# yoffy/libiqo

Hardware: AMD Instinct MI355X
Metric: Mpix/s Lanczos-3 U8 4K→1080p at 1/2/4/8 GPUs; achieved HBM GB/s %peak (higher is better)
Workload: dtype u8; 1 GPU; C2 Lanczos-3 U8 1ch 3840x2160->1920x1080; frames_per_gpu=1024, global_frames=1024, parallelism=image-sharded x1 (independent shards, no collective), kernel=lanczos_stream, bands_per_frame=auto, step=one libiqo_hip launch over the rank's device-resident batch

## Files before the change

### include/iqo_hip.h

```cpp
#ifndef IQO_HIP_H
#define IQO_HIP_H

#include <stddef.h>
#include <stdint.h>

#ifdef __cplusplus
extern "C" {
#endif

#define IQO_HIP_OK 0
#define IQO_HIP_EINVAL (-1)
#define IQO_HIP_ENODEV (-2)
#define IQO_HIP_ENOMEM (-3)
#define IQO_HIP_EHIP (-4)
#define IQO_HIP_EUNSUP (-5)

enum { IQO_METHOD_LANCZOS = 0, IQO_METHOD_AREA = 1, IQO_METHOD_LINEAR = 2 };

enum {
    IQO_KERNEL_GENERAL = 0,
    IQO_KERNEL_LANCZOS_STREAM = 1,
    IQO_KERNEL_AREA_INT = 2,
    IQO_KERNEL_LINEAR_UP2 = 3,
    IQO_KERNEL_TILE = 4,
// ... 145 lines not shown
int iqo_host_packed_kernel_for(int method, unsigned degree, int channels, size_t srcW, size_t srcH, size_t dstW,
                               size_t dstH, size_t pxScale);

enum {
    IQO_YUV420_NONE = 0,
    IQO_YUV420_LZ_SYMB10 = 1,
    IQO_YUV420_LZ_SYM10 = 2,
    IQO_YUV420_LZ_SYMB8 = 3,
    IQO_YUV420_LZ_SYM8 = 4,
    IQO_YUV420_AREA44 = 5,
    IQO_YUV420_AREA22 = 6,
    IQO_YUV420_AREA2Y = 7,
    IQO_YUV420_AREA4Y = 8,
    IQO_YUV420_AREA8Y = 9,
    IQO_YUV420_AREA33 = 10,
    IQO_YUV420_AREA3Y = 11,
    IQO_YUV420_AREA6Y = 12,
    IQO_YUV420_LIN_D2 = 13,
    IQO_YUV420_LIN_UP2 = 14
};

int iqo_host_yuv420_fused(int method, unsigned degree, size_t srcW, size_t srcH, size_t dstW, size_t dstH);

void iqo_dropin_backend_counts(int *hip, int *cpu);

#ifdef __cplusplus
}
#endif
#endif
```

### libiqo_amd/__init__.py

```python
import ctypes
import os

__all__ = ["IqoError", "LanczosResizer", "AreaResizer", "LinearResizer", "Yuv420Resizer", "Nv12Resizer", "available",
           "lib", "host_tables", "host_kernel_for", "host_packed_kernel_for", "host_yuv420_fused", "host_band_src_rows", "copy_frames", "ipc_export", "ipc_open",
           "ipc_close", "KERNELS", "YUV420_FUSED", "COPY_PATHS", "LIB_PATH", "Norm", "OUT_F32", "OUT_F16", "OUT_BF16",
           "CS_BT601_LIMITED", "CS_BT601_FULL", "CS_BT709_LIMITED", "CS_BT709_FULL", "COLOR_STANDARDS", "RGB_ORDERS",
           "host_yuv_to_rgb", "yuv_rgb_workspace_bytes", "CHROMA_REPLICATE", "CHROMA_FULL", "CHROMA_MODES",
           "host_chroma_full_kernel"]

PKG_DIR = os.path.dirname(os.path.abspath(__file__))
LIB_PATH = os.environ.get("LIBIQO_AMD_LIB") or os.path.join(PKG_DIR, "libiqo_hip.so")

KERNELS = {0: "general", 1: "lanczos_stream", 2: "area_int", 3: "linear_up2", 4: "tile", 5: "walk", 6: "lanczos_up2", 7: "lanczos_d32", 8: "area_d32", 9: "lanczos_u23", 10: "linear_u23", 11: "lanczos_d31", 12: "ryx", 13: "ryg", 14: "packed_tile", 15: "packed_general"}
YUV420_FUSED = {0: "none", 1: "lz_symb10", 2: "lz_sym10", 3: "lz_symb8", 4: "lz_sym8", 5: "area44", 6: "area22",
                7: "area2y", 8: "area4y", 9: "area8y", 10: "area33", 11: "area3y", 12: "area6y", 13: "lin_d2",
                14: "lin_up2"}
_METHODS = {"lanczos": 0, "area": 1, "linear": 2}

_c_sz = ctypes.c_size_t
_vp = ctypes.c_void_p


class IqoError(RuntimeError):
    pass


class PlanDesc(ctypes.Structure):
    _fields_ = [("method", ctypes.c_int), ("device", ctypes.c_int), ("srcW", _c_sz), ("srcH", _c_sz),
                ("dstW", _c_sz), ("dstH", _c_sz), ("tapsX", ctypes.c_int), ("tapsY", ctypes.c_int),
                ("phasesX", ctypes.c_int), ("phasesY", ctypes.c_int), ("kernel", ctypes.c_int),
                ("bandsPerFrame", ctypes.c_int), ("tileRows", ctypes.c_int)]


class Norm(ctypes.Structure):
    _fields_ = [("dtype", ctypes.c_int), ("planes", ctypes.c_int), ("order", ctypes.c_int * 4),
                ("scale", ctypes.c_float * 4), ("bias", ctypes.c_float * 4)]


OUT_F32, OUT_F16, OUT_BF16 = 1, 2, 3
CS_BT601_LIMITED, CS_BT601_FULL, CS_BT709_LIMITED, CS_BT709_FULL = 0, 1, 2, 3
COLOR_STANDARDS = {"bt601": CS_BT601_LIMITED, "bt601-full": CS_BT601_FULL, "bt709": CS_BT709_LIMITED,
                   "bt709-full": CS_BT709_FULL}
RGB_ORDERS = {"rgb": (0, 1, 2), "bgr": (2, 1, 0), "rgba": (0, 1, 2, 3), "bgra": (2, 1, 0, 3)}
CHROMA_REPLICATE, CHROMA_FULL = 0, 1
CHROMA_MODES = {"replicate": CHROMA_REPLICATE, "full": CHROMA_FULL}


class IpcHandle(ctypes.Structure):
    _fields_ = [("bytes", ctypes.c_ubyte * 64), ("offset", ctypes.c_uint64)]


COPY_PATHS = {0: "same device", 1: "peer DMA (xGMI)", 2: "host staging", 3: "host<->device"}

_lib = None
# ... 25 lines not shown
                                             _vp, _vp]
    L.iqo_hip_band_src_rows.argtypes = [_vp, _c_sz, _c_sz, ctypes.POINTER(_c_sz), ctypes.POINTER(_c_sz)]
    L.iqo_hip_resize_band.argtypes = [_vp, _c_sz, _c_sz, _c_sz, _c_sz, _c_sz, _c_sz, _vp, _c_sz, _c_sz, _vp, _vp]
    L.iqo_hip_strerror.restype = ctypes.c_char_p
    L.iqo_hip_strerror.argtypes = [ctypes.c_int]
    L.iqo_hip_version.restype = ctypes.c_char_p
    L.iqo_host_tables.argtypes = [ctypes.c_int, ctypes.c_uint, _c_sz, _c_sz, _c_sz, _c_sz, _c_sz, ctypes.c_int,
                                  ctypes.POINTER(ctypes.c_int), ctypes.POINTER(ctypes.c_int),
                                  ctypes.POINTER(ctypes.c_int32), _c_sz]
    L.iqo_host_kernel_for.argtypes = [ctypes.c_int, ctypes.c_uint, _c_sz, _c_sz, _c_sz, _c_sz, _c_sz]
    L.iqo_host_kernel_for_layout.argtypes = L.iqo_host_kernel_for.argtypes + [_c_sz, _c_sz]
    L.iqo_host_band_src_rows.argtypes = [ctypes.c_int, ctypes.c_uint, _c_sz, _c_sz, _c_sz, _c_sz, _c_sz, _c_sz, _c_sz,
                                         ctypes.POINTER(_c_sz), ctypes.POINTER(_c_sz)]
    L.iqo_hip_plan_yuv420.argtypes = [ctypes.c_int, ctypes.c_uint, _c_sz, _c_sz, _c_sz, _c_sz, ctypes.c_int, pp]
    L.iqo_hip_yuv_plan_destroy.argtypes = [_vp]
    L.iqo_hip_yuv_plan_destroy.restype = None
    L.iqo_hip_yuv_plane.argtypes = [_vp, ctypes.c_int]
    L.iqo_hip_yuv_plane.restype = _vp
    L.iqo_hip_resize_yuv420_device.argtypes = [_vp, _c_sz, _c_sz, _c_sz, _c_sz, _vp, _vp, _vp, _c_sz, _c_sz, _c_sz,
                                               _vp, _vp, _vp, _vp, ctypes.POINTER(ctypes.c_int)]
    L.iqo_hip_resize_yuv420.argtypes = [_vp, _c_sz, _vp, _c_sz, _vp, _vp, _c_sz, _vp, _c_sz, _vp, _vp]
    L.iqo_host_packed_kernel_for.argtypes = [ctypes.c_int, ctypes.c_uint, ctypes.c_int, _c_sz, _c_sz, _c_sz, _c_sz, _c_sz]
    L.iqo_host_yuv420_fused.argtypes = [ctypes.c_int, ctypes.c_uint, _c_sz, _c_sz, _c_sz, _c_sz]
    L.iqo_hip_plan_nv12.argtypes = [ctypes.c_int, ctypes.c_uint, _c_sz, _c_sz, _c_sz, _c_sz, ctypes.c_int, pp]
    L.iqo_hip_nv12_plan_destroy.argtypes = [_vp]
    L.iqo_hip_nv12_plan_destroy.restype = None
    L.iqo_hip_nv12_plane.argtypes = [_vp, ctypes.c_int]
    L.iqo_hip_nv12_plane.restype = _vp
    L.iqo_hip_resize_nv12_device.argtypes = [_vp, _c_sz, _c_sz, _c_sz, _c_sz, _vp, _vp, _c_sz, _c_sz, _c_sz, _vp, _vp,
                                             _vp]
    src_nv12 = [_vp, _c_sz, _c_sz, _c_sz, _c_sz, _vp, _vp]
    src_i420 = src_nv12 + [_vp]
    to_rgb = [ctypes.c_int, ctypes.c_int, ctypes.POINTER(ctypes.c_int), _c_sz, _c_sz, _vp, _vp, _c_sz, _vp]
    to_norm = [ctypes.c_int, ctypes.POINTER(Norm), _c_sz, _c_sz, _c_sz, _vp, _vp, _c_sz, _vp]
    L.iqo_hip_yuv_rgb_workspace_bytes.argtypes = [_c_sz, _c_sz, _c_sz]
    L.iqo_hip_yuv_rgb_workspace_bytes.restype = _c_sz
    L.iqo_hip_resize_nv12_rgb_device.argtypes = src_nv12 + to_rgb
    L.iqo_hip_resize_nv12_norm_device.argtypes = src_nv12 + to_norm
    L.iqo_hip_resize_yuv420_rgb_device.argtypes = src_i420 + to_rgb + [ctypes.POINTER(ctypes.c_int)]
    L.iqo_hip_resize_yuv420_norm_device.argtypes = src_i420 + to_norm + [ctypes.POINTER(ctypes.c_int)]
    L.iqo_host_yuv_to_rgb.argtypes = [ctypes.c_int, _c_sz, _vp, _vp, _vp, _vp]
    L.iqo_hip_yuv_rgb_workspace_bytes_chroma.argtypes = [_c_sz, _c_sz, _c_sz, ctypes.c_int]
    L.iqo_hip_yuv_rgb_workspace_bytes_chroma.restype = _c_sz
    for name in ("iqo_hip_nv12_plan_set_chroma", "iqo_hip_yuv_plan_set_chroma"):
        getattr(L, name).argtypes = [_vp, ctypes.c_int]
    for name in ("iqo_hip_nv12_plan_chroma", "iqo_hip_yuv_plan_chroma"):
# ... 64 lines not shown
    return a.value, b.value


def host_kernel_for(method, degree, srcW, srcH, dstW, dstH, pxScale=1, src_align=16, dst_align=16):
    k = lib().iqo_host_kernel_for_layout(_METHODS[method], degree, srcW, srcH, dstW, dstH, pxScale, src_align,
                                         dst_align)
    if k < 0:
        raise IqoError("invalid plan request")
    return KERNELS[k]


def host_packed_kernel_for(method, degree, channels, srcW, srcH, dstW, dstH, pxScale=1):
    k = lib().iqo_host_packed_kernel_for(_METHODS[method], degree, channels, srcW, srcH, dstW, dstH, pxScale)
    if k < 0:
        raise IqoError("invalid packed plan request")
    return KERNELS[k]


def host_yuv420_fused(method, degree, srcW, srcH, dstW, dstH):
    k = lib().iqo_host_yuv420_fused(_METHODS[method], degree, srcW, srcH, dstW, dstH)
    if k < 0:
        raise IqoError("invalid yuv420 plan request")
    return YUV420_FUSED[k]


def _standard(standard):
    if isinstance(standard, str):
        if standard not in COLOR_STANDARDS:
            raise IqoError("standard must be one of %s" % ", ".join(sorted(COLOR_STANDARDS)))
        return COLOR_STANDARDS[standard]
    return int(standard)


def _chroma(chroma):
    if not isinstance(chroma, str) or chroma not in CHROMA_MODES:
        raise IqoError("chroma must be one of %s" % ", ".join(sorted(CHROMA_MODES)))
    return CHROMA_MODES[chroma]


def yuv_rgb_workspace_bytes(dstW, dstH, nFrames, chroma="replicate"):
    return int(lib().iqo_hip_yuv_rgb_workspace_bytes_chroma(dstW, dstH, nFrames, _chroma(chroma)))


def host_chroma_full_kernel(method, degree, srcW, srcH, dstW, dstH, layout="nv12"):
    if layout not in ("nv12", "i420"):
        raise IqoError("layout must be nv12 or i420")
# ... 473 lines not shown
```

### libiqo_amd/csrc/abi.hip

```cpp
#include "iqo_hip.h"

#include <hip/hip_runtime.h>

#include <algorithm>
#include <cassert>
#include <cmath>
#include <cstdio>
#include <cstdlib>
#include <cstring>
#include <limits>
#include <condition_variable>
#include <mutex>
#include <new>
#include <thread>
#include <string>
#include <vector>

#include "kernels.hpp"
#include "plan.hpp"

using iqo_amd::AxisPlan;
using iqo_amd::CoordInfo;
using iqo_amd::Plan;

struct iqo_hip_plan;
namespace {
void reset_options(iqo_hip_plan *h);
}

struct iqo_hip_plan {
    iqo_hip_plan() { reset_options(this); }
    Plan p;
    int device = 0;
    int keyMethod = 0;
    unsigned keyDegree = 0;
    size_t keyDims[5] = {0, 0, 0, 0, 0};
    int channels = 1;
    iqo_amd::PackedTables pk;
    int4 *dPSpans = nullptr;
    std::vector<uint8_t> blob;
    std::vector<std::pair<void **, size_t>> blobPtrs;
    uint8_t *dBlob = nullptr;
    bool tablesUp = false;
    std::mutex tablesMu;
    int4 *dX = nullptr, *dY = nullptr, *dChunks = nullptr;
    int *dTabX = nullptr, *dTabY = nullptr;
    int nChunks = 0, ldsInts = 0;
    int forceGeneral, bands, hostStage, tail, rounds, ryxSplit, ryxAdj, ryxCpt, ryxUc, rygCpt, stack, prefetch,
        streamVariant, lanes, ratioPrefetch, chunkFrames;
    int useTile, useWalk, useUp2, useD32, useD31, useA32, useU23, useL23, useRyx, useRyg, useRyu, useRyuRun;
    int debugFlags;
#ifdef IQO_VARIANT_DEBUG
    uint64_t traceAddr;
#endif
    iqo_amd::TileTables tt;
    int tileTH0 = 0, tileSrcRows0 = 0;
    int4 *dTRows = nullptr, *dTSpans = nullptr;
    int2 *dTCols = nullptr;
    uint2 *dTRowTap = nullptr;
    uint32_t *dTColCoef = nullptr;
    int32_t *dTColA = nullptr;
    int tileNQp = 0;
    iqo_amd::WalkTables wt;
    iqo_amd::Up2Tables ut;
    iqo_amd::D32Tables dt;
    iqo_amd::D31Tables t31;
    iqo_amd::RyxTables ryx;
    uint32_t *dRyxRowCoef = nullptr, *dRyxColCoef = nullptr;
    int4 *dRyxCols = nullptr;
    int4 *dRyxRowRec = nullptr;
    int4 *dRyuPos = nullptr;
    int ryuBase = 0;
// ... 339 lines not shown
        if (hi - lo > kChunkLds)
            return IQO_HIP_EUNSUP;
        int xe = x + 1;
        while (xe < p.dstW && xe - x < kChunkOut) {
            int a, b;
            column_span(p, xe, &a, &b);
            int nlo = std::min(lo, a), nhi = std::max(hi, b);
            if (nhi - nlo > kChunkLds)
                break;
            lo = nlo;
            hi = nhi;
            ++xe;
        }
        chunks->push_back(make_int4(x, xe, lo, hi));
        *ldsInts = std::max(*ldsInts, hi - lo);
        x = xe;
    }
    return IQO_HIP_OK;
}

void free_plan(iqo_hip_plan *h)
{
    (void)hipFree(h->dBlob);
    delete h;
}

std::vector<int4> coord_records(const AxisPlan &a)
{
    std::vector<int4> v(a.coord.size());
    for (size_t i = 0; i < v.size(); ++i)
        v[i] = make_int4(a.coord[i].srcO, a.coord[i].tabOff, a.coord[i].kind, a.coord[i].aux);
    return v;
}

iqo_amd::RyxDev ryx_dev(const iqo_hip_plan *h);

void build_host_tables(iqo_hip_plan *h)
{
    iqo_amd::build_tile_tables(h->p, &h->tt);
    h->tileTH0 = h->tt.TH;
    h->tileSrcRows0 = h->tt.srcRows;
    if (h->tt.ok)
        iqo_amd::build_walk_tables(h->p, h->tt, &h->wt);
    iqo_amd::build_up2(h->p, h->wt, &h->ut);
    iqo_amd::build_d32(h->p, h->wt, &h->dt);
    iqo_amd::build_d31(h->p, &h->t31);
    iqo_amd::build_ryx(h->p, &h->ryx);
// ... 109 lines not shown
void stage_packed(iqo_hip_plan *h)
{
    std::vector<int4> spans(h->pk.spans.size());
    for (size_t i = 0; i < spans.size(); ++i)
        spans[i] = make_int4(h->pk.spans[i].lo8, h->pk.spans[i].groups, h->pk.spans[i].border, 0);
    upload(h, &h->dPSpans, spans.data(), spans.size());
}

struct Option {
    const char *name;
    int iqo_hip_plan::*member;
    long lo, hi;
    int def;
    bool pub;
};
using PlanT = iqo_hip_plan;
constexpr long kMax = std::numeric_limits<long>::max();
constexpr Option onoff(const char *name, int PlanT::*member, int def, bool pub) { return {name, member, 1, 0, def, pub}; }
constexpr Option kOptions[] = {
    onoff("force_general", &PlanT::forceGeneral, 0, true),
    {"bands", &PlanT::bands, 0, kMax, 0, true},
    {"host_stage", &PlanT::hostStage, 0, 1, 0, true},
    {"tail", &PlanT::tail, -1, 4096, 0, false},
    {"rounds", &PlanT::rounds, -1, 64, 0, false},
    {"ryx_split", &PlanT::ryxSplit, 0, 4, 1, false},
    {"ryx_adj", &PlanT::ryxAdj, 0, 1, 1, false},
    {"ryx_cpt", &PlanT::ryxCpt, 0, 1, 1, false},
    onoff("ryx_uc", &PlanT::ryxUc, 1, false),
    {"ryg_cpt", &PlanT::rygCpt, 0, 4, 0, false},
    {"stack", &PlanT::stack, 0, 2, 1, false},
    {"prefetch", &PlanT::prefetch, 1, 4, 3, false},
    {"stream_variant", &PlanT::streamVariant, 0, 2, 0, false},
    {"lanes", &PlanT::lanes, 0, 62, 0, false},
    {"ratio_prefetch", &PlanT::ratioPrefetch, 0, 8, 0, false},
    {"chunk_frames", &PlanT::chunkFrames, 0, kMax, 0, false},
    onoff("tile", &PlanT::useTile, 1, false),
    onoff("walk", &PlanT::useWalk, 1, false),
    onoff("up2", &PlanT::useUp2, 1, false),
    onoff("d32", &PlanT::useD32, 1, false),
    onoff("d31", &PlanT::useD31, 1, false),
    onoff("a32", &PlanT::useA32, 1, false),
    onoff("u23", &PlanT::useU23, 1, false),
    onoff("l23", &PlanT::useL23, 1, false),
    onoff("ryx", &PlanT::useRyx, 1, false),
    onoff("ryg", &PlanT::useRyg, 1, false),
    onoff("ryu", &PlanT::useRyu, 1, false),
// ... 742 lines not shown
    if (h->chunkFrames > 0) {
        chunk = std::min(chunk, static_cast<size_t>(h->chunkFrames));
        const size_t n = (nFrames + chunk - 1) / chunk;
        chunk = (nFrames + n - 1) / n;
    }
    if (h->ratioPrefetch > 0) {
        const int pd = h->ratioPrefetch;
        bool ok = true;
        if (kernel == IQO_KERNEL_LANCZOS_D32)
            ok = h->dt.variant == 0 ? (pd == 1 || pd == 2 || pd == 4) : (pd == 1 || pd == 3);
        else if (kernel == IQO_KERNEL_LANCZOS_D31)
            ok = h->t31.variant == 0 ? (pd == 1 || pd == 5) : (pd == 1 || pd == 2 || pd == 4);
        else if (kernel == IQO_KERNEL_LANCZOS_U23 || kernel == IQO_KERNEL_LINEAR_U23)
            ok = pd == 1 || pd == 2;
        else if (kernel == IQO_KERNEL_AREA_D32)
            ok = pd == 2 || pd == 4 || pd == 8;
        if (!ok)
            return IQO_HIP_EINVAL;
    }
    for (size_t f0 = 0; f0 < nFrames; f0 += chunk) {
        const iqo_amd::Io io = make_io(std::min(chunk, nFrames - f0), src + f0 * srcFrameSt, srcSt, srcFrameSt, srcRow0,
                                       s1, dst + f0 * dstFrameSt, dstSt, dstFrameSt, rb);
        hipError_t e = hipSuccess;
        if (kernel == IQO_KERNEL_LANCZOS_STREAM)
            e = iqo_amd::launch_lanczos_stream(lanczos_dev(h), io, rb, re, h->bands, s);
        else if (kernel == IQO_KERNEL_AREA_INT)
            e = iqo_amd::launch_area_int(area_dev(h), io, rb, re, s);
        else if (kernel == IQO_KERNEL_LINEAR_UP2)
            e = iqo_amd::launch_linear_up2(linear_dev(h), io, rb, re, h->bands, s);
        else if (kernel == IQO_KERNEL_TILE)
            e = iqo_amd::launch_tile(tile_dev(h), io, rb, re, s);
        else if (kernel == IQO_KERNEL_WALK)
            e = iqo_amd::launch_walk(walk_dev(h), io, rb, re, h->bands, s);
        else if (kernel == IQO_KERNEL_LANCZOS_UP2)
            e = iqo_amd::launch_up2(up2_dev(h), io, rb, re, h->bands, s);
        else if (kernel == IQO_KERNEL_LANCZOS_D32)
            e = iqo_amd::launch_d32(d32_dev(h), io, rb, re, h->bands, s);
        else if (kernel == IQO_KERNEL_LANCZOS_D31)
            e = iqo_amd::launch_d31(d31_dev(h), io, rb, re, h->bands, s);
        else if (kernel == IQO_KERNEL_RYX)
            e = iqo_amd::launch_ryx(ryx_dev(h), io, rb, re, h->bands, s);
        else if (kernel == IQO_KERNEL_RYG)
            e = iqo_amd::launch_ryg(ryg_dev(h), io, rb, re, h->bands, s);
        else if (kernel == IQO_KERNEL_AREA_D32)
            e = iqo_amd::launch_a32(a32_dev(h), io, rb, re, h->bands, s);
        else if (kernel == IQO_KERNEL_LANCZOS_U23)
            e = iqo_amd::launch_u23(u23_dev(h), io, rb, re, h->bands, s);
        else if (kernel == IQO_KERNEL_LINEAR_U23)
            e = iqo_amd::launch_l23(l23_dev(h), io, rb, re, h->bands, s);
// ... 139 lines not shown
    d->method = h->p.method;
    d->device = h->device;
    d->srcW = static_cast<size_t>(h->p.srcW);
    d->srcH = static_cast<size_t>(h->p.srcH);
    d->dstW = static_cast<size_t>(h->p.dstW);
    d->dstH = static_cast<size_t>(h->p.dstH);
    d->tapsX = h->p.x.taps;
    d->tapsY = h->p.y.taps;
    d->phasesX = h->p.x.phases;
    d->phasesY = h->p.y.phases;
    d->kernel = plan_kernel(h);
    d->bandsPerFrame = h->bands;
    d->tileRows = h->channels > 1 ? (h->pk.ok ? h->pk.TH : 0) : h->tt.ok ? h->tt.TH : 0;
    return IQO_HIP_OK;
}

int iqo_hip_plan_prepare(iqo_hip_plan *h)
{
    if (!h)
        return IQO_HIP_EINVAL;
    DeviceGuard guard(h->device);
    if (!guard.ok())
        return IQO_HIP_ENODEV;
    return ensure_tables(h);
}

bool tuning_enabled()
{
    const char *e = std::getenv("IQO_HIP_TUNING");
    return e && *e && std::strcmp(e, "0") != 0;
}

int iqo_hip_plan_set_option(iqo_hip_plan *h, const char *key, long value)
{
    if (!h || !key)
        return IQO_HIP_EINVAL;
    const Option *o = std::find_if(std::begin(kOptions), std::end(kOptions),
                                   [&](const Option &r) { return !std::strcmp(key, r.name); });
    const bool known = o != std::end(kOptions);
    if (!(known && o->pub) && !tuning_enabled())
        return IQO_HIP_EINVAL;
    if (known) {
        const bool onoff = o->lo > o->hi;
        if (!onoff && (value < o->lo || value > o->hi))
            return IQO_HIP_EINVAL;
        if (o->member == &iqo_hip_plan::rygCpt && value == 1)
// ... 1136 lines not shown
                      int(IQO_YUV420_LIN_UP2) + 1 == int(iqo_amd::kYuvFusedCount),
                  "iqo_hip.h IQO_YUV420_* are kernels.hpp Yuv420Fused");
    if (method < 0 || method > 2 || srcW < 2 || srcH < 2 || dstW < 2 || dstH < 2)
        return IQO_HIP_EINVAL;
    const iqo_amd::Method m = static_cast<iqo_amd::Method>(method);
    iqo_hip_plan hy, hc;
    std::string err;
    if (!iqo_amd::build_plan(m, degree, srcW, srcH, dstW, dstH, 1, &hy.p, &err) ||
        !iqo_amd::build_plan(m, degree, srcW / 2, srcH / 2, dstW / 2, dstH / 2, m == iqo_amd::kLanczos ? 2 : 1, &hc.p,
                             &err))
        return IQO_HIP_EINVAL;
    const int k = hy.p.kernel;
    if (k != hc.p.kernel)
        return IQO_YUV420_NONE;
    if (k == IQO_KERNEL_LANCZOS_STREAM)
        return iqo_amd::yuv420_fused(lanczos_dev(&hy), lanczos_dev(&hc)).label;
    if (k == IQO_KERNEL_AREA_INT)
        return iqo_amd::yuv420_fused(area_dev(&hy), area_dev(&hc)).label;
    if (k == IQO_KERNEL_LINEAR_UP2)
        return iqo_amd::yuv420_fused(linear_dev(&hy), linear_dev(&hc)).label;
    return IQO_YUV420_NONE;
}

}
```

### libiqo_amd/csrc/kernels.hip

```cpp
#include "kernels_dev.hpp"

namespace iqo_amd {
namespace {


enum { KMAIN = 0, KLO = 1, KHI = 2, KID = 3 };

struct GeneralArgs {
    GeneralDev g;
    Io io;
    int rowBegin;
};

__device__ __forceinline__ int src_px(const GeneralArgs &a, const uint8_t *srcF, int row, int col)
{
    return srcF[static_cast<int64_t>(row - a.io.srcRow0) * a.io.srcSt + col];
}

__device__ int y_value(const GeneralArgs &a, const uint8_t *srcF, int4 yi, int col)
{
    const GeneralDev &g = a.g;
    if (g.method == 0) {
        if (yi.z == KID)
            return static_cast<int16_t>(static_cast<uint16_t>(src_px(a, srcF, yi.x, col) * 64));
// ... 301 lines not shown
            __builtin_amdgcn_raw_buffer_store_b32(o, dstR, off, 0, 0);
        } else {
#pragma unroll
            for (int k = 0; k < 4; ++k)
                if (x0 + k < t.dstW)
                    __builtin_amdgcn_raw_buffer_store_b8(static_cast<uint8_t>(bytes[k]), dstR, off + k, 0, 0);
        }
    }
}


struct LanczosArgs {
    LanczosDev l;
    Io io;
    int rowBegin, rowEnd, rowsPerBand;
    int srcBytes, dstBytes;
    int bands, wavesPerRow;
    int dbg;
    int np;
    int rowPitch, chunks;
    int lastLanes;
    int fpw, frames;
    int tailBands, tailRows, framesPerXcd;
};

template <int KY, int KX, int NY, int NXP, int OFFXD, int PD>
__device__ __forceinline__ void lanczos_stream_kernel_body(const LanczosArgs &a, const unsigned bx, const unsigned by)
{
    constexpr int OUTS = 16 / KX;
    constexpr int OPW = 62 * OUTS;
    constexpr int P = NY / KY;
    static_assert(NY % KY == 0, "NY must be a multiple of KY");
    constexpr int LV = P * PD / cgcd(P, PD);
    constexpr int DLO = OFFXD;
    constexpr int DHI = (OUTS - 1) * KX / 2 + OFFXD + NXP / 2;
    static_assert(DLO >= -8 && DHI <= 16, "horizontal taps must stay within the neighbouring lanes");
    static_assert(OUTS == 8, "edge handling assumes 8 outputs per lane (KX == 2)");

    const LanczosDev &L = a.l;
    const int lane = static_cast<int>(threadIdx.x) & 63;
    const int wib = __builtin_amdgcn_readfirstlane(static_cast<int>(threadIdx.x) >> 6);
    const int g = static_cast<int>(bx) * 4 + wib;
    if (g >= a.bands * a.wavesPerRow)
        return;
    const int band = g / a.wavesPerRow, wcol = g - band * a.wavesPerRow;
    const int y0 = a.rowBegin + band * a.rowsPerBand;
    const int y1 = min(y0 + a.rowsPerBand, a.rowEnd);
// ... 758 lines not shown
            if (edgeR && laneR)
                edgeSum[1][slot] = make_int4(sum[4], sum[5], sum[6], sum[7]);
            if (slot == EB - 1 || i == nRows - 1) {
                __builtin_amdgcn_wave_barrier();
                flush_edges(yy - dir * slot, slot + 1);
            }
        }
    };
    for (int base = 0; base < nRows; base += H)
        static_for<H>([&](auto uc) { row(uc, base); });
    if (LINE && (edgeL || edgeR) && nRows % H) {
        const int baseLast = nRows - nRows % H;
        __builtin_amdgcn_wave_barrier();
        flush_lines(dir > 0 ? y0 + baseLast : y1 - 1 - baseLast, nRows % H);
    }

    wait_vmcnt<0>();
}
template <int NY, int NX, int OFFX, int K, int CPW, bool C0ONE, bool LINE>
__global__ __launch_bounds__(256) __attribute__((amdgpu_waves_per_eu(NY > 12 ? 2 : NY > 10 ? 3 : 4))) void lanczos_symb_kernel(LanczosArgs a)
{
    unsigned bx = blockIdx.x, by = blockIdx.y;
    int rpb = a.rowsPerBand;
    if (a.tailBands > 0) {
        const int x = static_cast<int>(blockIdx.x & 7u), idx = static_cast<int>(blockIdx.x >> 3);
        const int F8 = a.framesPerXcd, nLong = (F8 - 1) * a.bands;
        const bool inter = !(IQO_DBG(a) & 128);
        if (idx < nLong) {
            const int q = idx / a.bands;
            by = static_cast<unsigned>(inter ? 8 * q + x : x * F8 + q);
            bx = static_cast<unsigned>(idx - q * a.bands);
        } else {
            by = static_cast<unsigned>(inter ? 8 * (F8 - 1) + x : x * F8 + F8 - 1);
            bx = static_cast<unsigned>(idx - nLong);
            rpb = a.tailRows;
            if (static_cast<int>(bx) >= a.tailBands)
                return;
        }
    } else {
        const unsigned bands = gridDim.x;
        const unsigned lg = xcd_chunks(by * bands + bx, bands, bands * gridDim.y);
        by = lg / bands;
        bx = lg - by * bands;
    }
#ifdef IQO_VARIANT_DEBUG
    uint32_t t0 = 0;
    if (a.l.trace && threadIdx.x < 64)
        t0 = static_cast<uint32_t>(__builtin_amdgcn_s_memrealtime());
#endif
    lanczos_symb_kernel_body<NY, NX, OFFX, K, CPW, C0ONE, LINE>(a, bx, by, rpb);
#ifdef IQO_VARIANT_DEBUG
    if (a.l.trace && threadIdx.x == 0) {
        const uint32_t t1 = static_cast<uint32_t>(__builtin_amdgcn_s_memrealtime());
        const uint32_t hw = static_cast<uint32_t>(__builtin_amdgcn_s_getreg(4 | (31 << 11)));
        const uint32_t xcc = static_cast<uint32_t>(__builtin_amdgcn_s_getreg(20 | (31 << 11)));
        uint4 *rec = reinterpret_cast<uint4 *>(a.l.trace) + (blockIdx.x + gridDim.x * blockIdx.y);
        *rec = make_uint4(t0, t1, hw, xcc);
    }
#endif
}


template <int NY, int NX, int OFFX, int K, int CPW, bool C0ONE>
__global__ __launch_bounds__(128) __attribute__((amdgpu_waves_per_eu(4))) void lanczos_stack_kernel(LanczosArgs a)
{
    constexpr int H = NY / 2;
    static_assert(NY % 2 == 0 && NX % 2 == 0 && (OFFX & 1), "even taps, odd first X column");
    static_assert(K == H && CPW >= 1, "ring depth = window period");
    constexpr int WAIT = 1 + (K - 2) * (2 * CPW + 1);
    constexpr int WAITLA = 1 + (K - 3) * (2 * CPW + 1);
    constexpr int JLO = (OFFX + 1) / 2;
    constexpr int EB = 16;
    constexpr int PITCH = 2048;
    constexpr int SLOT = 2 * PITCH;
    constexpr int OOB = 0x7ff00000;
    extern __shared__ __attribute__((aligned(16))) uint8_t lds[];
    uint8_t *const ring = lds;
    int4 *const edgeSum = reinterpret_cast<int4 *>(lds + K * SLOT);
    const uint32_t sinkLds = static_cast<uint32_t>(K * SLOT + 2 * CPW * 2 * EB * 16);

// ... 978 lines not shown
}



bool lanczos_stream_supported(int KY, int KX, int NY, int NXP, int offX)
{
    return KY == 2 && KX == 2 &&
           ((NY == 10 && NXP == 14 && offX == -6) || (NY == 8 && NXP == 10 && offX == -4) ||
            (NY == 4 && NXP == 4 && offX == 0));
}

int lanczos_stream_block(int) { return 256; }

template <typename A>
struct Prep {
    A a;
    dim3 grid;
    int block = 256, lds = 0;
    const void *kern = nullptr;
    int kind = 0;
    int pd = 0;
};

hipError_t prep_lanczos(const LanczosDev &l, const Io &io, int rowBegin, int rowEnd, int bands, Prep<LanczosArgs> *P)
{
    const int rows = rowEnd - rowBegin;
    int opw = 62 * (16 / l.KX);
    int wpr = (l.dstW + opw - 1) / opw;
    int np = 62;
    if (l.sym) {
        const int lanes = (l.dstW + 7) / 8;
        np = l.np > 0 ? min(l.np, 62) : (lanes + wpr - 1) / wpr;
        if (np * 8 > l.dstW)
            np = l.dstW / 8;
        if (l.NY >= 12 && ((l.dstW + 8 * np - 1) / (8 * np) > 4 || (l.NY == 16 && !symb_line(l.dstW, np))))
            np = (lanes + wpr - 1) / wpr;
        opw = 8 * np;
        wpr = (l.dstW + opw - 1) / opw;
    }
    const int pd = l.prefetch;
    const void *kern = nullptr;
    int block = 256, ldsBytes = 0;
    const int rowNeed = (std::max(32 + 2 * l.dstW, 16 + l.srcW) + 15) & ~15;
    const int chunks = (rowNeed - 16 + 1023) / 1024;
    const int lastLanes = (rowNeed - 16 - 1024 * (chunks - 1)) / 16;
    const int cpw = (chunks + wpr - 1) / wpr;
    const bool shared = l.sym == 1 && wpr <= 4 && cpw <= 2;
// ... 62 lines not shown
        if (l.NY == 10 && one)
            kern = pd <= 2 ? reinterpret_cast<const void *>(lanczos_sym_kernel<10, 12, -5, 3, true>)
                           : reinterpret_cast<const void *>(lanczos_sym_kernel<10, 12, -5, 4, true>);
        else if (l.NY == 10)
            kern = reinterpret_cast<const void *>(lanczos_sym_kernel<10, 12, -5, 4, false>);
        else
            kern = pd <= 2 ? reinterpret_cast<const void *>(lanczos_sym_kernel<8, 8, -3, 3, false>)
                           : reinterpret_cast<const void *>(lanczos_sym_kernel<8, 8, -3, 4, false>);
    } else if (l.NY == 4) {
        kern = pd <= 1   ? reinterpret_cast<const void *>(lanczos_stream_kernel<2, 2, 4, 4, 0, 1>)
               : pd == 2 ? reinterpret_cast<const void *>(lanczos_stream_kernel<2, 2, 4, 4, 0, 2>)
                         : reinterpret_cast<const void *>(lanczos_stream_kernel<2, 2, 4, 4, 0, 3>);
    } else if (l.NY == 10) {
        kern = pd <= 1   ? reinterpret_cast<const void *>(lanczos_stream_kernel<2, 2, 10, 14, -3, 1>)
               : pd == 2 ? reinterpret_cast<const void *>(lanczos_stream_kernel<2, 2, 10, 14, -3, 2>)
                         : reinterpret_cast<const void *>(lanczos_stream_kernel<2, 2, 10, 14, -3, 3>);
    } else {
        kern = pd <= 1   ? reinterpret_cast<const void *>(lanczos_stream_kernel<2, 2, 8, 10, -2, 1>)
               : pd == 2 ? reinterpret_cast<const void *>(lanczos_stream_kernel<2, 2, 8, 10, -2, 2>)
                         : reinterpret_cast<const void *>(lanczos_stream_kernel<2, 2, 8, 10, -2, 3>);
    }
    const int groups = stack ? (io.frames + fpw - 1) / fpw : io.frames;
    if (bands <= 0) {
        const int resident = resident_waves(kern, block, ldsBytes);
        if (stack) {
            const int64_t want = static_cast<int64_t>(l.rounds > 0 ? l.rounds : 6) * (resident / 2);
            bands = static_cast<int>(std::min<int64_t>((want + groups - 1) / groups, std::max(1, rows / 16)));
        } else if (shared && l.rounds >= 0) {
            const int64_t want = static_cast<int64_t>(l.rounds > 0 ? l.rounds : 6) * (resident / wpr);
            const int64_t byRounds = (want + io.frames - 1) / io.frames;
            const int rowsMax = l.NY <= 10 ? (l.dstW >= 640 ? (l.NY == 10 ? 15 : 12) : 24)
                                           : std::min(48, std::max(22, 22 * 1920 / std::max(1, l.dstW)));
            const int rowsMin = l.NY <= 10 ? 12 : 16;
            bands = static_cast<int>(std::min<int64_t>(std::max<int64_t>(byRounds, (rows + rowsMax - 1) / rowsMax),
                                                       std::max(1, rows / rowsMin)));
        } else {
            bands = choose_bands(rows, io.frames, wpr, resident, l.NY - 2);
        }
    }
    bands = max(1, min(bands, rows));
    const int rpb = (rows + bands - 1) / bands;
    bands = (rows + rpb - 1) / rpb;
    LanczosArgs &a = P->a;
    a = LanczosArgs{l, io, rowBegin, rowEnd, rpb, 0, 0, bands, wpr, l.dbg, np, rowPitch, chunks,
                    pack ? lastLanes : 64, fpw, io.frames, 0, 0, 0};
    if (shared && !stack && l.tail >= 0 && io.frames % 8 == 0 && io.frames >= 16) {
        const int tb = l.tail > 0 ? min(l.tail, rows) : (rows + 7) / 8;
        const int tr = (rows + tb - 1) / tb;
        a.tailBands = (rows + tr - 1) / tr;
        a.tailRows = tr;
        a.framesPerXcd = io.frames / 8;
        if (a.tailBands <= bands)
            a.tailBands = 0;
    }
    const int64_t sb = static_cast<int64_t>(io.srcRowEnd - io.srcRow0 - 1) * io.srcSt + l.srcW;
    const int64_t db = static_cast<int64_t>(rowEnd - 1 - io.dstRow0) * io.dstSt + l.dstW;
    if (sb >= (int64_t(1) << 31) || db >= (int64_t(1) << 31) || io.srcSt >= (int64_t(1) << 31) ||
        io.dstSt >= (int64_t(1) << 31))
        return hipErrorInvalidValue;
    a.srcBytes = static_cast<int>(sb);
    a.dstBytes = static_cast<int>(db);
    const int waves = bands * wpr;
    P->grid = shared ? dim3(static_cast<unsigned>(bands), static_cast<unsigned>(groups))
                       : dim3(static_cast<unsigned>((waves + 3) / 4), static_cast<unsigned>(io.frames));
    if (a.tailBands > 0)
        P->grid = dim3(static_cast<unsigned>(8 * ((a.framesPerXcd - 1) * bands + a.tailBands)), 1u);
    P->block = block;
    P->lds = ldsBytes;
    P->kern = kern;
    P->kind = stack ? 3 : shared ? 1 : (l.sym ? 2 : 0);
    P->pd = pd;
    return hipSuccess;
}

hipError_t launch_lanczos_stream(const LanczosDev &l, const Io &io, int rowBegin, int rowEnd, int bands,
                                 hipStream_t s)
{
    if (rowEnd <= rowBegin || io.frames <= 0)
        return hipSuccess;
    Prep<LanczosArgs> P;
    hipError_t e = prep_lanczos(l, io, rowBegin, rowEnd, bands, &P);
    if (e != hipSuccess)
        return e;
    void *args[] = {&P.a};
    return hipLaunchKernel(P.kern, P.grid, dim3(static_cast<unsigned>(P.block)), args, static_cast<size_t>(P.lds), s);
}

constexpr int kAreaKinds = 9;
int area_kind(const AreaDev &g)
{
    if (g.lin)
        return 8;
    if (g.KX == 3)
        return g.KY == 3 ? 5 : 6;
    if (g.KX == 6)
        return 7;
    return g.KX == 4 && g.KY == 4 ? 0 : g.KX == 2 && g.KY == 2 ? 1 : g.KX == 2 ? 2 : g.KX == 4 ? 3 : 4;
}

hipError_t prep_area(const AreaDev &g, const Io &io, int rowBegin, int rowEnd, Prep<AreaArgs> *P)
{
    const int cols = 16 % g.KX == 0 ? 16 : 12;
    P->a = AreaArgs{g, io, rowBegin, rowEnd, g.srcW / cols};
    const int64_t total = static_cast<int64_t>(rowEnd - rowBegin) * P->a.groups;
    P->grid = dim3(static_cast<unsigned>((total + 255) / 256), static_cast<unsigned>(io.frames));
    P->kind = area_kind(g);
    static const void *const kerns[kAreaKinds] = {
        reinterpret_cast<const void *>(area_int_kernel<4, 4>), reinterpret_cast<const void *>(area_int_kernel<2, 2>),
// ... 236 lines not shown
```

### libiqo_amd/csrc/kernels.hpp

```cpp
#pragma once

#include <hip/hip_runtime.h>

#include <cstdint>

#include "colorspace.hpp"

namespace iqo_amd {

struct Io {
    const uint8_t *src;
    int64_t srcSt, srcFrameSt;
    int srcRow0;
    int srcRowEnd;
    uint8_t *dst;
    int64_t dstSt, dstFrameSt;
    int dstRow0;
    int frames;
};

struct GeneralDev {
    int method, srcW, srcH, dstW, nX, nY;
    const int4 *xInfo, *yInfo;
    const int *tabX, *tabY;
// ... 195 lines not shown
    int KY, KX, NY, NXP, offX;
    int srcW, srcH, dstW, dstH;
    int offY;
    uint32_t cy[16];
    uint32_t cx[16];
    int mainBeginY, mainEndY, mainBeginX, mainEndX;
    uint32_t yTopM[16], yBotM[16], xM[8];
    int yTopS[16], yBotS[16], xT[8];
    int yTopNeg, yBotNeg, xNeg;
    int dbg;
    int prefetch;
    int sym;
    int NX, offXO;
    uint32_t cxo[8];
    int np;
    int rounds;
    int stack;
    int tail;
#ifdef IQO_VARIANT_DEBUG
    uint64_t trace;
#endif
};
bool lanczos_stream_supported(int KY, int KX, int NY, int NXP, int offX);
hipError_t launch_lanczos_stream(const LanczosDev &l, const Io &io, int rowBegin, int rowEnd, int bands,
                                 hipStream_t s);
int lanczos_stream_block(int srcW);

struct AreaDev {
    int KY, KX, srcW, dstW, dstH;
    uint32_t cy[16];
    uint32_t cx[8];
    int lin;
    int srcH;
};
hipError_t launch_area_int(const AreaDev &a, const Io &io, int rowBegin, int rowEnd, hipStream_t s);

struct LinearDev {
    int srcW, srcH, dstW, dstH;
    int F;
    uint32_t cy[3];
    uint32_t cx[3];
    int dbg;
    int np;
};
hipError_t launch_linear_up2(const LinearDev &l, const Io &io, int rowBegin, int rowEnd, int bands,
                             hipStream_t s);

enum Yuv420Fused {
// ... 25 lines not shown
```

Measured before the change: 1.165 million Mpix/s.

## Add atomic-ticket work pool for tail frames in lanczos stream kernel

```diff
diff --git a/include/iqo_hip.h b/include/iqo_hip.h
--- a/include/iqo_hip.h
+++ b/include/iqo_hip.h
@@ -191,6 +191,14 @@
 
 int iqo_host_yuv420_fused(int method, unsigned degree, size_t srcW, size_t srcH, size_t dstW, size_t dstH);
 
+typedef struct iqo_stream_band {
+    int xcd, frame, row0, rows;
+} iqo_stream_band;
+int iqo_host_streamer_schedule(int method, unsigned degree, size_t srcW, size_t srcH, size_t dstW, size_t dstH,
+                               size_t nFrames, int bands, int tail, int tailFrames, int tailExtra, int residentWaves,
+                               iqo_stream_band *statics, size_t statCap, size_t *nStatic, iqo_stream_band *pool,
+                               size_t poolCap, size_t *nPool, size_t *poolBlocks);
+
 void iqo_dropin_backend_counts(int *hip, int *cpu);
 
 #ifdef __cplusplus
diff --git a/libiqo_amd/__init__.py b/libiqo_amd/__init__.py
--- a/libiqo_amd/__init__.py
+++ b/libiqo_amd/__init__.py
@@ -2,7 +2,7 @@
 import os
 
 __all__ = ["IqoError", "LanczosResizer", "AreaResizer", "LinearResizer", "Yuv420Resizer", "Nv12Resizer", "available",
-           "lib", "host_tables", "host_kernel_for", "host_packed_kernel_for", "host_yuv420_fused", "host_band_src_rows", "copy_frames", "ipc_export", "ipc_open",
+           "lib", "host_tables", "host_kernel_for", "host_packed_kernel_for", "host_yuv420_fused", "host_streamer_schedule", "host_band_src_rows", "copy_frames", "ipc_export", "ipc_open",
            "ipc_close", "KERNELS", "YUV420_FUSED", "COPY_PATHS", "LIB_PATH", "Norm", "OUT_F32", "OUT_F16", "OUT_BF16",
            "CS_BT601_LIMITED", "CS_BT601_FULL", "CS_BT709_LIMITED", "CS_BT709_FULL", "COLOR_STANDARDS", "RGB_ORDERS",
            "host_yuv_to_rgb", "yuv_rgb_workspace_bytes", "CHROMA_REPLICATE", "CHROMA_FULL", "CHROMA_MODES",
@@ -30,6 +30,10 @@
                 ("dstW", _c_sz), ("dstH", _c_sz), ("tapsX", ctypes.c_int), ("tapsY", ctypes.c_int),
                 ("phasesX", ctypes.c_int), ("phasesY", ctypes.c_int), ("kernel", ctypes.c_int),
                 ("bandsPerFrame", ctypes.c_int), ("tileRows", ctypes.c_int)]
+
+
+class StreamBand(ctypes.Structure):
+    _fields_ = [("xcd", ctypes.c_int), ("frame", ctypes.c_int), ("row0", ctypes.c_int), ("rows", ctypes.c_int)]
 
 
 class Norm(ctypes.Structure):
@@ -101,6 +105,8 @@
     L.iqo_hip_resize_yuv420.argtypes = [_vp, _c_sz, _vp, _c_sz, _vp, _vp, _c_sz, _vp, _c_sz, _vp, _vp]
     L.iqo_host_packed_kernel_for.argtypes = [ctypes.c_int, ctypes.c_uint, ctypes.c_int, _c_sz, _c_sz, _c_sz, _c_sz, _c_sz]
     L.iqo_host_yuv420_fused.argtypes = [ctypes.c_int, ctypes.c_uint, _c_sz, _c_sz, _c_sz, _c_sz]
+    L.iqo_host_streamer_schedule.argtypes = [ctypes.c_int, ctypes.c_uint, _c_sz, _c_sz, _c_sz, _c_sz, _c_sz] + \
+        [ctypes.c_int] * 5 + [ctypes.POINTER(StreamBand), _c_sz, ctypes.POINTER(_c_sz)] * 2 + [ctypes.POINTER(_c_sz)]
     L.iqo_hip_plan_nv12.argtypes = [ctypes.c_int, ctypes.c_uint, _c_sz, _c_sz, _c_sz, _c_sz, ctypes.c_int, pp]
     L.iqo_hip_nv12_plan_destroy.argtypes = [_vp]
     L.iqo_hip_nv12_plan_destroy.restype = None
@@ -211,6 +217,21 @@
     if k < 0:
         raise IqoError("invalid yuv420 plan request")
     return YUV420_FUSED[k]
+
+
+def host_streamer_schedule(degree, srcW, srcH, dstW, dstH, frames, bands=0, tail=0, tail_frames=-1, tail_extra=0,
+                           resident_waves=0):
+    L = lib()
+    ns, npool, nb = _c_sz(), _c_sz(), _c_sz()
+    head = (_METHODS["lanczos"], degree, srcW, srcH, dstW, dstH, frames, bands, tail, tail_frames, tail_extra,
+            resident_waves)
+    _check(L.iqo_host_streamer_schedule(*head, None, 0, ctypes.byref(ns), None, 0, ctypes.byref(npool),
+                                        ctypes.byref(nb)), "host_streamer_schedule")
+    st, po = (StreamBand * max(1, ns.value))(), (StreamBand * max(1, npool.value))()
+    _check(L.iqo_host_streamer_schedule(*head, st, ns.value, ctypes.byref(ns), po, npool.value, ctypes.byref(npool),
+                                        ctypes.byref(nb)), "host_streamer_schedule")
+    rec = lambda a, n: [(b.xcd, b.frame, b.row0, b.rows) for b in a[:n]]
+    return {"static": rec(st, ns.value), "pool": rec(po, npool.value), "pool_blocks": nb.value}
 
 
 def _standard(standard):
diff --git a/libiqo_amd/csrc/abi.hip b/libiqo_amd/csrc/abi.hip
--- a/libiqo_amd/csrc/abi.hip
+++ b/libiqo_amd/csrc/abi.hip
@@ -14,6 +14,7 @@
 #include <new>
 #include <thread>
 #include <string>
+#include <unordered_map>
 #include <vector>
 
 #include "kernels.hpp"
@@ -46,8 +47,12 @@
     int4 *dX = nullptr, *dY = nullptr, *dChunks = nullptr;
     int *dTabX = nullptr, *dTabY = nullptr;
     int nChunks = 0, ldsInts = 0;
-    int forceGeneral, bands, hostStage, tail, rounds, ryxSplit, ryxAdj, ryxCpt, ryxUc, rygCpt, stack, prefetch,
-        streamVariant, lanes, ratioPrefetch, chunkFrames;
+    int forceGeneral, bands, hostStage, tail, tailFrames, tailExtra, rounds, ryxSplit, ryxAdj, ryxCpt, ryxUc, rygCpt, stack,
+        prefetch, streamVariant, lanes, ratioPrefetch, chunkFrames;
+    std::mutex poolMu;
+    std::vector<uint32_t *> poolSlabs;
+    size_t poolUsed = 0;
+    std::unordered_map<hipStream_t, uint32_t *> poolOfStream;
     int useTile, useWalk, useUp2, useD32, useD31, useA32, useU23, useL23, useRyx, useRyg, useRyu, useRyuRun;
     int debugFlags;
 #ifdef IQO_VARIANT_DEBUG
@@ -433,7 +438,42 @@
 void free_plan(iqo_hip_plan *h)
 {
     (void)hipFree(h->dBlob);
+    for (uint32_t *slab : h->poolSlabs)
+        (void)hipFree(slab);
     delete h;
+}
+
+constexpr size_t kPoolSlab = 256;
+uint32_t *pool_counter(iqo_hip_plan *h, hipStream_t s)
+{
+    hipStreamCaptureStatus cs = hipStreamCaptureStatusNone;
+    const bool capturing = s && hipStreamIsCapturing(s, &cs) == hipSuccess && cs == hipStreamCaptureStatusActive;
+    std::lock_guard<std::mutex> lock(h->poolMu);
+    if (!capturing) {
+        auto it = h->poolOfStream.find(s);
+        if (it != h->poolOfStream.end())
+            return it->second;
+    }
+    if (h->poolSlabs.empty() || h->poolUsed == kPoolSlab) {
+        static const uint32_t zeros[kPoolSlab] = {};
+        hipStreamCaptureMode mode = hipStreamCaptureModeRelaxed;
+        (void)hipThreadExchangeStreamCaptureMode(&mode);
+        uint32_t *slab = nullptr;
+        bool ok = hipMalloc(reinterpret_cast<void **>(&slab), sizeof zeros) == hipSuccess;
+        if (ok && hipMemcpy(slab, zeros, sizeof zeros, hipMemcpyHostToDevice) != hipSuccess) {
+            (void)hipFree(slab);
+            ok = false;
+        }
+        (void)hipThreadExchangeStreamCaptureMode(&mode);
+        if (!ok)
+            return nullptr;
+        h->poolSlabs.push_back(slab);
+        h->poolUsed = 0;
+    }
+    uint32_t *c = h->poolSlabs.back() + h->poolUsed++;
+    if (!capturing)
+        h->poolOfStream.emplace(s, c);
+    return c;
 }
 
 std::vector<int4> coord_records(const AxisPlan &a)
@@ -589,6 +629,8 @@
     {"bands", &PlanT::bands, 0, kMax, 0, true},
     {"host_stage", &PlanT::hostStage, 0, 1, 0, true},
     {"tail", &PlanT::tail, -1, 4096, 0, false},
+    {"tail_frames", &PlanT::tailFrames, -1, 4096, -1, false},
+    {"tail_extra", &PlanT::tailExtra, 0, 1000, 0, false},
     {"rounds", &PlanT::rounds, -1, 64, 0, false},
     {"ryx_split", &PlanT::ryxSplit, 0, 4, 1, false},
     {"ryx_adj", &PlanT::ryxAdj, 0, 1, 1, false},
@@ -1377,9 +1419,17 @@
         const iqo_amd::Io io = make_io(std::min(chunk, nFrames - f0), src + f0 * srcFrameSt, srcSt, srcFrameSt, srcRow0,
                                        s1, dst + f0 * dstFrameSt, dstSt, dstFrameSt, rb);
         hipError_t e = hipSuccess;
-        if (kernel == IQO_KERNEL_LANCZOS_STREAM)
-            e = iqo_amd::launch_lanczos_stream(lanczos_dev(h), io, rb, re, h->bands, s);
-        else if (kernel == IQO_KERNEL_AREA_INT)
+        if (kernel == IQO_KERNEL_LANCZOS_STREAM) {
+            iqo_amd::StreamPool pool;
+            const int m = h->tailFrames < 0 ? iqo_amd::stream_pool_frames_auto(io.frames) : h->tailFrames;
+            if (m > 0 && h->tail >= 0 && rb == 0 && re == p.dstH && io.frames % 8 == 0 && io.frames >= 16) {
+                pool.frames = m;
+                pool.extraPct = h->tailExtra;
+                if (!(pool.counter = pool_counter(h, s)))
+                    return IQO_HIP_ENOMEM;
+            }
+            e = iqo_amd::launch_lanczos_stream(lanczos_dev(h), io, rb, re, h->bands, s, pool);
+        } else if (kernel == IQO_KERNEL_AREA_INT)
             e = iqo_amd::launch_area_int(area_dev(h), io, rb, re, s);
         else if (kernel == IQO_KERNEL_LINEAR_UP2)
             e = iqo_amd::launch_linear_up2(linear_dev(h), io, rb, re, h->bands, s);
@@ -1565,6 +1615,8 @@
     DeviceGuard guard(h->device);
     if (!guard.ok())
         return IQO_HIP_ENODEV;
+    if (plan_kernel(h) == IQO_KERNEL_LANCZOS_STREAM && !pool_counter(h, nullptr))
+        return IQO_HIP_ENOMEM;
     return ensure_tables(h);
 }
 
@@ -2747,4 +2799,48 @@
     return IQO_YUV420_NONE;
 }
 
-}
+int iqo_host_streamer_schedule(int method, unsigned degree, size_t srcW, size_t srcH, size_t dstW, size_t dstH,
+                               size_t nFrames, int bands, int tail, int tailFrames, int tailExtra, int residentWaves,
+                               iqo_stream_band *statics, size_t statCap, size_t *nStatic, iqo_stream_band *pool,
+                               size_t poolCap, size_t *nPool, size_t *poolBlocks)
+{
+    if (method != IQO_METHOD_LANCZOS || !nStatic || !nPool || !poolBlocks || nFrames == 0 || nFrames > 65535 || bands < 0 ||
+        tail < -1 || tail > 4096 || tailFrames < -1 || tailExtra < 0 || residentWaves < 0)
+        return IQO_HIP_EINVAL;
+    iqo_hip_plan h;
+    std::string err;
+    if (!iqo_amd::build_plan(iqo_amd::kLanczos, degree, srcW, srcH, dstW, dstH, 1, &h.p, &err))
+        return IQO_HIP_EINVAL;
+    if (h.p.kernel != IQO_KERNEL_LANCZOS_STREAM)
+        return IQO_HIP_EUNSUP;
+    h.tail = tail;
+    const int frames = static_cast<int>(nFrames);
+    const int m = tail < 0 ? 0 : tailFrames < 0 ? iqo_amd::stream_pool_frames_auto(frames) : tailFrames;
+    iqo_amd::StreamTail t;
+    if (!iqo_amd::stream_schedule(lanczos_dev(&h), frames, bands, m, tailExtra, residentWaves, &t))
+        return IQO_HIP_EUNSUP;
+    size_t ns = 0, np = 0;
+    auto put = [&](iqo_stream_band *out, size_t cap, size_t *n, int xcd, const iqo_amd::StreamBlock &b) {
+        const int row0 = b.band * b.rows;
+        if (out && *n < cap)
+            out[*n] = iqo_stream_band{xcd, b.frame, row0, std::min(b.rows, h.p.dstH - row0)};
+        ++*n;
+    };
+    if (t.tailBands == 0) {
+        for (int f = 0; f < frames; ++f)
+            for (int b = 0; b < t.bands; ++b)
+                put(statics, statCap, &ns, -1, iqo_amd::StreamBlock{f, b, t.rowsPerBand});
+    } else {
+        for (int x = 0; x < 8; ++x)
+            for (int i = 0; i < iqo_amd::stream_static_blocks(t); ++i)
+                put(statics, statCap, &ns, x, iqo_amd::stream_block(t, x, i));
+        for (int k = 0; k < iqo_amd::stream_pool_items(t); ++k)
+            put(pool, poolCap, &np, -1, iqo_amd::stream_pool_item(t, k));
+    }
+    *nStatic = ns;
+    *nPool = np;
+    *poolBlocks = static_cast<size_t>(8) * static_cast<size_t>(t.poolBlocks);
+    return IQO_HIP_OK;
+}
+
+}
diff --git a/libiqo_amd/csrc/kernels.hip b/libiqo_amd/csrc/kernels.hip
--- a/libiqo_amd/csrc/kernels.hip
+++ b/libiqo_amd/csrc/kernels.hip
@@ -347,7 +347,13 @@
     int lastLanes;
     int fpw, frames;
     int tailBands, tailRows, framesPerXcd;
+    int poolFrames;
+    uint32_t *poolCounter;
 };
+__host__ __device__ inline StreamTail stream_tail(const LanczosArgs &a, int poolBlocks)
+{
+    return StreamTail{a.bands, a.rowsPerBand, a.tailBands, a.tailRows, a.framesPerXcd, a.poolFrames, poolBlocks};
+}
 
 template <int KY, int KX, int NY, int NXP, int OFFXD, int PD>
 __device__ __forceinline__ void lanczos_stream_kernel_body(const LanczosArgs &a, const unsigned bx, const unsigned by)
@@ -1152,21 +1158,31 @@
 {
     unsigned bx = blockIdx.x, by = blockIdx.y;
     int rpb = a.rowsPerBand;
+    [[maybe_unused]] int ticket = -1;
     if (a.tailBands > 0) {
         const int x = static_cast<int>(blockIdx.x & 7u), idx = static_cast<int>(blockIdx.x >> 3);
-        const int F8 = a.framesPerXcd, nLong = (F8 - 1) * a.bands;
         const bool inter = !(IQO_DBG(a) & 128);
-        if (idx < nLong) {
-            const int q = idx / a.bands;
-            by = static_cast<unsigned>(inter ? 8 * q + x : x * F8 + q);
-            bx = static_cast<unsigned>(idx - q * a.bands);
-        } else {
-            by = static_cast<unsigned>(inter ? 8 * (F8 - 1) + x : x * F8 + F8 - 1);
-            bx = static_cast<unsigned>(idx - nLong);
-            rpb = a.tailRows;
-            if (static_cast<int>(bx) >= a.tailBands)
+        const StreamTail st = stream_tail(a, 0);
+        StreamBlock b = stream_block(st, x, idx, inter);
+        if (b.frame < 0) {
+            extern __shared__ __attribute__((aligned(16))) uint8_t lds[];
+            uint32_t *const slot = reinterpret_cast<uint32_t *>(lds + K * 2 * a.rowPitch);
+            if (threadIdx.x == 0) {
+                const uint32_t drawn = 8u * static_cast<uint32_t>(static_cast<int>(gridDim.x >> 3) - stream_static_blocks(st));
+                const uint32_t t = __hip_atomic_fetch_add(a.poolCounter, 1u, __ATOMIC_RELAXED, __HIP_MEMORY_SCOPE_AGENT);
+                if (t == drawn - 1u)
+                    __hip_atomic_store(a.poolCounter, 0u, __ATOMIC_RELAXED, __HIP_MEMORY_SCOPE_AGENT);
+                *slot = t;
+            }
+            __syncthreads();
+            ticket = __builtin_amdgcn_readfirstlane(static_cast<int>(*slot));
+            if (static_cast<uint32_t>(ticket) >= static_cast<uint32_t>(stream_pool_items(st)))
                 return;
-        }
+            b = stream_pool_item(st, ticket);
+        }
+        by = static_cast<unsigned>(b.frame);
+        bx = static_cast<unsigned>(b.band);
+        rpb = b.rows;
     } else {
         const unsigned bands = gridDim.x;
         const unsigned lg = xcd_chunks(by * bands + bx, bands, bands * gridDim.y);
@@ -1185,7 +1201,7 @@
         const uint32_t hw = static_cast<uint32_t>(__builtin_amdgcn_s_getreg(4 | (31 << 11)));
         const uint32_t xcc = static_cast<uint32_t>(__builtin_amdgcn_s_getreg(20 | (31 << 11)));
         uint4 *rec = reinterpret_cast<uint4 *>(a.l.trace) + (blockIdx.x + gridDim.x * blockIdx.y);
-        *rec = make_uint4(t0, t1, hw, xcc);
+        *rec = make_uint4(t0, t1, hw, (xcc & 0xfu) | (static_cast<uint32_t>(ticket + 1) << 4));
     }
 #endif
 }
@@ -2210,7 +2226,15 @@
     int pd = 0;
 };
 
-hipError_t prep_lanczos(const LanczosDev &l, const Io &io, int rowBegin, int rowEnd, int bands, Prep<LanczosArgs> *P)
+constexpr int kPoolBandRows = 12;
+constexpr int kPoolExtraPct = 50;
+int stream_pool_frames_auto(int frames)
+{
+    return frames >= 1024 ? 2 : frames >= 256 ? 1 : 0;
+}
+
+hipError_t prep_lanczos(const LanczosDev &l, const Io &io, int rowBegin, int rowEnd, int bands, Prep<LanczosArgs> *P,
+                        const StreamPool &pool = StreamPool(), int residentWaves = 0)
 {
     const int rows = rowEnd - rowBegin;
     int opw = 62 * (16 / l.KX);
@@ -2319,7 +2343,7 @@
     }
     const int groups = stack ? (io.frames + fpw - 1) / fpw : io.frames;
     if (bands <= 0) {
-        const int resident = resident_waves(kern, block, ldsBytes);
+        const int resident = residentWaves > 0 ? residentWaves : resident_waves(kern, block, ldsBytes);
         if (stack) {
             const int64_t want = static_cast<int64_t>(l.rounds > 0 ? l.rounds : 6) * (resident / 2);
             bands = static_cast<int>(std::min<int64_t>((want + groups - 1) / groups, std::max(1, rows / 16)));
@@ -2340,15 +2364,30 @@
     bands = (rows + rpb - 1) / rpb;
     LanczosArgs &a = P->a;
     a = LanczosArgs{l, io, rowBegin, rowEnd, rpb, 0, 0, bands, wpr, l.dbg, np, rowPitch, chunks,
-                    pack ? lastLanes : 64, fpw, io.frames, 0, 0, 0};
+                    pack ? lastLanes : 64, fpw, io.frames, 0, 0, 0, 0, nullptr};
+    const bool wantPool = pool.frames > 0 && pool.counter && rowBegin == 0 && rowEnd == l.dstH && !(IQO_DBG(l) & 128);
+    int poolBlocks = 0;
     if (shared && !stack && l.tail >= 0 && io.frames % 8 == 0 && io.frames >= 16) {
-        const int tb = l.tail > 0 ? min(l.tail, rows) : (rows + 7) / 8;
-        const int tr = (rows + tb - 1) / tb;
-        a.tailBands = (rows + tr - 1) / tr;
-        a.tailRows = tr;
+        auto split = [&](int tb) {
+            a.tailRows = (rows + tb - 1) / tb;
+            a.tailBands = (rows + a.tailRows - 1) / a.tailRows;
+        };
+        split(l.tail > 0 ? min(l.tail, rows) : (rows + (wantPool ? kPoolBandRows : 8) - 1) / (wantPool ? kPoolBandRows : 8));
+        if (wantPool && l.tail == 0 && a.tailBands <= bands)
+            split((rows + 7) / 8);
         a.framesPerXcd = io.frames / 8;
         if (a.tailBands <= bands)
             a.tailBands = 0;
+    }
+    if (a.tailBands > 0 && wantPool) {
+        a.poolFrames = min(pool.frames, a.framesPerXcd);
+        a.poolCounter = pool.counter;
+        const int64_t items = stream_pool_items(stream_tail(a, 0));
+        const int64_t pct = 100 + (pool.extraPct > 0 ? pool.extraPct : kPoolExtraPct);
+        const int64_t per = (items * pct + 799) / 800;
+        if (8 * ((a.framesPerXcd - a.poolFrames) * static_cast<int64_t>(bands) + per) >= (int64_t(1) << 31))
+            return hipErrorInvalidValue;
+        poolBlocks = static_cast<int>(per);
     }
     const int64_t sb = static_cast<int64_t>(io.srcRowEnd - io.srcRow0 - 1) * io.srcSt + l.srcW;
     const int64_t db = static_cast<int64_t>(rowEnd - 1 - io.dstRow0) * io.dstSt + l.dstW;
@@ -2361,7 +2400,7 @@
     P->grid = shared ? dim3(static_cast<unsigned>(bands), static_cast<unsigned>(groups))
                        : dim3(static_cast<unsigned>((waves + 3) / 4), static_cast<unsigned>(io.frames));
     if (a.tailBands > 0)
-        P->grid = dim3(static_cast<unsigned>(8 * ((a.framesPerXcd - 1) * bands + a.tailBands)), 1u);
+        P->grid = dim3(static_cast<unsigned>(8 * (stream_static_blocks(stream_tail(a, 0)) + poolBlocks)), 1u);
     P->block = block;
     P->lds = ldsBytes;
     P->kern = kern;
@@ -2371,16 +2410,47 @@
 }
 
 hipError_t launch_lanczos_stream(const LanczosDev &l, const Io &io, int rowBegin, int rowEnd, int bands,
-                                 hipStream_t s)
+                                 hipStream_t s, const StreamPool &pool)
 {
     if (rowEnd <= rowBegin || io.frames <= 0)
         return hipSuccess;
     Prep<LanczosArgs> P;
-    hipError_t e = prep_lanczos(l, io, rowBegin, rowEnd, bands, &P);
+    hipError_t e = prep_lanczos(l, io, rowBegin, rowEnd, bands, &P, pool);
     if (e != hipSuccess)
         return e;
     void *args[] = {&P.a};
     return hipLaunchKernel(P.kern, P.grid, dim3(static_cast<unsigned>(P.block)), args, static_cast<size_t>(P.lds), s);
+}
+
+bool stream_schedule(const LanczosDev &l, int frames, int bands, int poolFrames, int extraPct, int residentWaves,
+                     StreamTail *out)
+{
+    Io io{};
+    io.srcSt = l.srcW;
+    io.srcFrameSt = static_cast<int64_t>(l.srcW) * l.srcH;
+    io.srcRowEnd = l.srcH;
+    io.dstSt = l.dstW;
+    io.dstFrameSt = static_cast<int64_t>(l.dstW) * l.dstH;
+    io.frames = frames;
+    static uint32_t never;
+    Prep<LanczosArgs> P;
+    if (frames <= 0)
+        return false;
+    if (residentWaves <= 0) {
+        if (prep_lanczos(l, io, 0, l.dstH, 1, &P) != hipSuccess || P.kind != 1)
+            return false;
+        const int wavesPerWg = P.block / 64, wavesPerCu = 4 * (l.NY > 12 ? 2 : l.NY > 10 ? 3 : 4);
+        residentWaves = 256 * wavesPerWg * std::max(1, std::min(wavesPerCu / wavesPerWg, 163840 / std::max(1, P.lds)));
+    }
+    if (prep_lanczos(l, io, 0, l.dstH, bands, &P, StreamPool{poolFrames, extraPct, &never}, residentWaves) != hipSuccess ||
+        P.kind != 1)
+        return false;
+    const StreamTail st = stream_tail(P.a, 0);
+    *out = st;
+    out->poolBlocks = P.a.tailBands > 0 ? static_cast<int>(P.grid.x / 8) - stream_static_blocks(st) : 0;
+    if (P.a.tailBands == 0)
+        out->framesPerXcd = out->poolFrames = 0;
+    return true;
 }
 
 constexpr int kAreaKinds = 9;
diff --git a/libiqo_amd/csrc/kernels.hpp b/libiqo_amd/csrc/kernels.hpp
--- a/libiqo_amd/csrc/kernels.hpp
+++ b/libiqo_amd/csrc/kernels.hpp
@@ -241,8 +241,46 @@
 #endif
 };
 bool lanczos_stream_supported(int KY, int KX, int NY, int NXP, int offX);
+
+struct StreamTail {
+    int bands, rowsPerBand;
+    int tailBands, tailRows;
+    int framesPerXcd;
+    int poolFrames, poolBlocks;
+};
+struct StreamBlock {
+    int frame, band, rows;
+};
+__host__ __device__ inline int stream_static_blocks(const StreamTail &t)
+{
+    return t.poolFrames > 0 ? (t.framesPerXcd - t.poolFrames) * t.bands : (t.framesPerXcd - 1) * t.bands + t.tailBands;
+}
+__host__ __device__ inline int stream_pool_items(const StreamTail &t) { return 8 * t.poolFrames * t.tailBands; }
+__host__ __device__ inline StreamBlock stream_block(const StreamTail &t, int x, int idx, bool interleaved = true)
+{
+    const int F8 = t.framesPerXcd, nLong = (F8 - (t.poolFrames > 0 ? t.poolFrames : 1)) * t.bands;
+    if (idx < nLong) {
+        const int q = idx / t.bands;
+        return StreamBlock{interleaved ? 8 * q + x : x * F8 + q, idx - q * t.bands, t.rowsPerBand};
+    }
+    if (t.poolFrames > 0)
+        return StreamBlock{-1, 0, 0};
+    return StreamBlock{interleaved ? 8 * (F8 - 1) + x : x * F8 + F8 - 1, idx - nLong, t.tailRows};
+}
+__host__ __device__ inline StreamBlock stream_pool_item(const StreamTail &t, int ticket)
+{
+    const int f = ticket / t.tailBands;
+    return StreamBlock{8 * (t.framesPerXcd - t.poolFrames) + f, ticket - f * t.tailBands, t.tailRows};
+}
+struct StreamPool {
+    int frames = 0, extraPct = 0;
+    uint32_t *counter = nullptr;
+};
+bool stream_schedule(const LanczosDev &l, int frames, int bands, int poolFrames, int extraPct, int residentWaves,
+                     StreamTail *out);
+int stream_pool_frames_auto(int frames);
 hipError_t launch_lanczos_stream(const LanczosDev &l, const Io &io, int rowBegin, int rowEnd, int bands,
-                                 hipStream_t s);
+                                 hipStream_t s, const StreamPool &pool = StreamPool());
 int lanczos_stream_block(int srcW);
 
 struct AreaDev {
```

After: 1.175 million Mpix/s (median of 6 runs). About the same (+0.8%).
